# wgurecky/bipymc

Hardware: AMD Instinct MI355X
Metric: chain-updates/sec (higher is better)
Workload: dtype f64

## Files before the change

### bipymc_amd/csrc/kernels.h

```cpp
#pragma once
#ifndef __HIPCC_RTC__
#include <hip/hip_runtime.h>
#include <stdint.h>
#endif

#include "philox.h"

#ifdef BPM_STAMPS
#define BPM_STAMP(i)                                                                          \
    do {                                                                                      \
        __builtin_amdgcn_sched_barrier(0);                                                    \
        unsigned long long _t;                                                                \
        asm volatile("s_memtime %0\n\ts_waitcnt lgkmcnt(0)" : "=s"(_t)::"memory");            \
        __builtin_amdgcn_sched_barrier(0);                                                    \
        bpm_stamp[i] = _t;                                                                    \
    } while (0)
#else
#define BPM_STAMP(i) do { } while (0)
#endif

#if defined(__HIP_DEVICE_COMPILE__) && !defined(__gfx942__) && !defined(__gfx950__)
#error "kernels.h: the ticket hand-overs rely on gfx942 / gfx950 memory behaviour (vmcnt counts stores; agent-scope atomics bypass the L2s): use __ATOMIC_RELEASE / __ATOMIC_ACQUIRE tickets on other targets"
#endif

// ... 459 lines not shown
        }
    }
}

template <int LPC, int DPL>
__device__ __forceinline__ void store_row_sys(double* row, int q, uint32_t ld, const double* v) {
#pragma unroll
    for (int u = 0; u < DPL / 2; ++u) {
        const uint32_t pi = (uint32_t)(q + u * LPC);
        if (2 * pi < ld) {
            __hip_atomic_store(row + 2 * pi, v[2 * u], __ATOMIC_RELAXED, __HIP_MEMORY_SCOPE_SYSTEM);
            __hip_atomic_store(row + 2 * pi + 1, v[2 * u + 1], __ATOMIC_RELAXED, __HIP_MEMORY_SCOPE_SYSTEM);
        }
    }
}

template <int LPC, int DPL>
__device__ __forceinline__ void store_row_stream(double* row, int q, uint32_t ld, const double* v) {
#pragma unroll
    for (int u = 0; u < DPL / 2; ++u) {
        const uint32_t pi = (uint32_t)(q + u * LPC);
        if (2 * pi < ld) {
            bpm_d2v t = {v[2 * u], v[2 * u + 1]};
            __builtin_nontemporal_store(t, reinterpret_cast<bpm_d2v*>(row) + pi);
        }
    }
}

__device__ __forceinline__ void box_muller_pair_f32(uint32_t w1, uint32_t w2, double& n0, double& n1) {
    const float u1 = ((float)w1 + 1.0f) * 2.3283064365386963e-10f;
    const float u2 = (float)w2 * 2.3283064365386963e-10f;
    const float r = __builtin_amdgcn_sqrtf(-2.0f * 0.6931471805599453f * __builtin_amdgcn_logf(u1));
    n0 = (double)(r * __builtin_amdgcn_cosf(u2));
    n1 = (double)(r * __builtin_amdgcn_sinf(u2));
}

template <int K>
__device__ __forceinline__ uint32_t quad_bcast(uint32_t v) {
    return (uint32_t)__builtin_amdgcn_update_dpp(0, (int)v, K * 0x55, 0xF, 0xF, false);
}

template <int LPC, int NPART_CT>
struct Partners {
    uint32_t r[NPART_CT > 0 ? NPART_CT : 1];
    const uint32_t* lds;
    __device__ __forceinline__ uint32_t get(int i) const { return NPART_CT > 0 ? r[i] : lds[i]; }
};

__device__ __forceinline__ uint32_t partner_pos(const PhaseArgs& a, uint32_t c, uint32_t idx, uint32_t n_pair_idx) {
    if (idx < n_pair_idx) {
        const uint32_t p = idx >> 1;
        const u32x4 wb = chain_block(a.seed, c, a.t, SLOT_PAIR0 + (p >> 1));
        uint32_t ia, ib;
        distinct_pair((p & 1) ? wb.z : wb.x, (p & 1) ? wb.w : wb.y, a.M, ia, ib);
        uint32_t pos = (idx & 1) ? ib : ia;
        if (a.mode == 2) pos += (pos >= c) ? 1u : 0u;
        return pos;
    }
    const u32x4 ws = chain_block(a.seed, c, a.t, SLOT_SNK);
    uint32_t iz, i1, i2;
    distinct_three(ws.x, ws.y, ws.z, a.M, iz, i1, i2);
    const uint32_t s = idx - n_pair_idx;
    return s == 0 ? iz : (s == 1 ? i1 : i2);
}

__device__ __forceinline__ uint32_t pos_to_chain(const PhaseArgs& a, uint32_t pos) {
#if defined(BPM_TEST_HOOKS) && defined(BPM_FAKE_NO_PARTNER_HOP)
    return pos;
#else
    return a.perm_tab ? a.perm_tab[pos] : perm_fwd(pos, a.pk);
#endif
}
__device__ __forceinline__ uint32_t own_pos_to_chain(const PhaseArgs& a, uint32_t pos) {
#if defined(BPM_TEST_HOOKS) && defined(BPM_FAKE_NO_OWN_HOP)
    return pos;
#else
    return a.perm_tab ? a.perm_tab[pos] : perm_fwd(pos, a.pk);
#endif
}
__device__ __forceinline__ uint32_t chain_to_pos(const PhaseArgs& a, uint32_t c) {
    return a.inv_tab ? a.inv_tab[c] : perm_inv(c, a.pk);
}

struct NoEarly { template <class W> __device__ __forceinline__ void operator()(W&) const {} };
struct PcrGiven { bool on = false; double p[MAX_CR]; };
template <int ALGO, int LPC, int DPL, int NP, int LOAD_LL = 1 , class EARLY = NoEarly>
__device__ __forceinline__ void make_proposal(const PhaseArgs& a, uint32_t c, bool active, int q, int cw,
                                              uint32_t* s_part, Work<DPL>& wk, const uint32_t* rec = nullptr,
                                              unsigned long long* bpm_stamp = nullptr, EARLY early = EARLY(), const PcrGiven pcr_ovr = PcrGiven()) {
    constexpr bool DREAM = ALGO == ALGO_DREAM;
    constexpr bool FAST = (NP > 0) && (LPC == 1);
    constexpr bool SNK_DIRECT = (LPC == 1);
    const uint32_t dim = a.L.dim, ld = a.L.ld;
    const uint32_t P = NP > 0 ? (uint32_t)NP : a.P;
    load_row<LPC, DPL>(row_ptr(a.L, c), q, ld, wk.x);
    wk.ll_cur = 0.0;
    wk.acc_prev = 0u;
    if (!a.replay) {
#if defined(BPM_TEST_HOOKS) && defined(BPM_FAKE_NO_LL)
        if (LPC < WAVE) wk.ll_cur = wk.x[0] * 1e-300; else
#endif
        if (LOAD_LL == 1 || (LOAD_LL == 2 && !a.lean)) wk.ll_cur = a.ll[c - a.lo];
        if (LPC == WAVE) wk.acc_prev = a.acc_count[c - a.lo];
    }
    if (DREAM && a.adapt_on) {
        load_row<LPC, DPL>(a.w_mean + (uint32_t)((c - a.lo) * 2u * ld), q, ld, wk.w_mean);
        load_row<LPC, DPL>(a.w_m2 + (uint32_t)((c - a.lo) * 2u * ld), q, ld, wk.w_m2);
    }
    double pcr[MAX_CR];
    if (DREAM) {
#pragma unroll
        for (int m = 0; m < MAX_CR; ++m) pcr[m] = pcr_ovr.on ? pcr_ovr.p[m] : a.cr_state[m];
    }
    double gtab[DPL];
    if (DREAM && LPC == WAVE) {
#pragma unroll
        for (int u = 0; u < DPL; ++u) {
            const uint32_t gi = (uint32_t)(q + u * WAVE);
            const double gl = a.gamma_tab[gi <= dim ? gi : dim];
            gtab[u] = gi <= dim ? gl : 0.0;
        }
    }
    double gt_lane = 0.0;
    if (DREAM && LPC * DPL < WAVE) {
        const uint32_t wl = (uint32_t)threadIdx.x & (uint32_t)(WAVE - 1);
        gt_lane = a.gamma_tab[wl <= dim ? wl : dim];
    }
    const bool snk_possible = !DREAM && a.p_snooker > 0.0 && a.M >= 3;
    const uint32_t npart = 2 * P + (snk_possible ? 3u : 0u);
    constexpr bool RL = (LPC == WAVE) && (NP > 0) && !FAST;
    const uint32_t npairs = (dim + 1u) >> 1;
    const bool merged = RL && DPL == 2 && (npairs + 2u * (uint32_t)NP + 1u <= (uint32_t)WAVE);
    u32x4 wpair[DPL / 2];
    u32x4 h0;
    constexpr bool QUAD = DREAM && LPC == 4 && DPL == 2 && NP == 3;
    constexpr bool REGS = FAST || RL || QUAD;
    Partners<LPC, REGS ? 2 * NP : 0> part;
    part.lds = s_part + cw * MAX_PARTNERS;
    const bool planned = (LPC == WAVE) && rec != nullptr;
    const bool dims_late = planned && RL && DPL == 2;
    if (planned) {
        h0.x = rec[1]; h0.y = rec[2]; h0.z = rec[3]; h0.w = rec[4];
        if (FAST || RL) {
#pragma unroll
            for (int i = 0; i < 2 * NP; ++i) part.r[i] = rec[5 + i];
        }
        if (!dims_late) {
#pragma unroll
            for (int u = 0; u < DPL / 2; ++u) wpair[u] = chain_block(a.seed, c, a.t, SLOT_DIM0 + (uint32_t)(q + u * LPC));
        }
    } else if (merged) {
        const uint32_t uq = (uint32_t)q, hdr_lane = npairs + 2u * (uint32_t)NP;
        const uint32_t pidx = uq - npairs;
        const uint32_t slot = uq < npairs ? SLOT_DIM0 + uq : (uq < hdr_lane ? SLOT_PAIR0 + (pidx >> 2) : SLOT_HDR0);
        const u32x4 wb = chain_block(a.seed, c, a.t, slot);
        wpair[0] = wb;
        h0.x = (uint32_t)__builtin_amdgcn_readlane((int)wb.x, hdr_lane);
        h0.y = (uint32_t)__builtin_amdgcn_readlane((int)wb.y, hdr_lane);
        h0.z = (uint32_t)__builtin_amdgcn_readlane((int)wb.z, hdr_lane);
        h0.w = (uint32_t)__builtin_amdgcn_readlane((int)wb.w, hdr_lane);
        BPM_STAMP(2);
        uint32_t mine = 0;
        if (uq >= npairs && uq < hdr_lane) {
            const uint32_t p = pidx >> 1;
            uint32_t ia, ib;
            distinct_pair((p & 1) ? wb.z : wb.x, (p & 1) ? wb.w : wb.y, a.M, ia, ib);
            uint32_t pos = (pidx & 1) ? ib : ia;
            if (a.mode == 2) pos += (pos >= c) ? 1u : 0u;
            mine = pos_to_chain(a, a.pool_off + pos);
        }
#pragma unroll
        for (int i = 0; i < 2 * NP; ++i) part.r[i] = (uint32_t)__builtin_amdgcn_readlane((int)mine, npairs + i);
    } else if (QUAD) {
        wpair[0] = chain_block(a.seed, c, a.t, SLOT_DIM0 + (uint32_t)q);
        const u32x4 wb = chain_block(a.seed, c, a.t, q == 1 ? SLOT_PAIR0 : (q == 2 ? SLOT_PAIR0 + 1u : SLOT_HDR0));
        h0.x = quad_bcast<0>(wb.x); h0.y = quad_bcast<0>(wb.y); h0.z = quad_bcast<0>(wb.z); h0.w = quad_bcast<0>(wb.w);
        uint32_t i0 = 0, i1 = 0, i2 = 0, i3 = 0;
        if (q == 1 || q == 2) {
            uint32_t ia, ib;
            distinct_pair(wb.x, wb.y, a.M, ia, ib);
            i0 = pos_to_chain(a, a.pool_off + ia); i1 = pos_to_chain(a, a.pool_off + ib);
            if (q == 1) {
                distinct_pair(wb.z, wb.w, a.M, ia, ib);
                i2 = pos_to_chain(a, a.pool_off + ia); i3 = pos_to_chain(a, a.pool_off + ib);
            }
        }
        part.r[0] = quad_bcast<1>(i0); part.r[1] = quad_bcast<1>(i1); part.r[2] = quad_bcast<1>(i2); part.r[3] = quad_bcast<1>(i3);
        part.r[4] = quad_bcast<2>(i0); part.r[5] = quad_bcast<2>(i1);
    } else {
        h0 = chain_block(a.seed, c, a.t, SLOT_HDR0);
#pragma unroll
        for (int u = 0; u < DPL / 2; ++u) wpair[u] = chain_block(a.seed, c, a.t, SLOT_DIM0 + (uint32_t)(q + u * LPC));
        if (FAST) {
#pragma unroll
            for (int i = 0; i < 2 * NP; ++i) part.r[i] = pos_to_chain(a, a.pool_off + partner_pos(a, c, (uint32_t)i, 2u * NP));
        }
        if (RL) {
            uint32_t mine = 0;
            if (q < 2 * NP) mine = pos_to_chain(a, a.pool_off + partner_pos(a, c, (uint32_t)q, 2u * NP));
#pragma unroll
            for (int i = 0; i < 2 * NP; ++i) part.r[i] = (uint32_t)__builtin_amdgcn_readlane((int)mine, i);
        }
    }
    BPM_STAMP(3);
    wk.u_acc = u01_53(h0.z, h0.w);
    const double u_sel = (double)(h0.x >> 16) * 1.52587890625e-05;
    const double u_gam = (double)(h0.x & 0xFFFFu) * 1.52587890625e-05;
    uint32_t snk_id[3] = {0u, 0u, 0u};
    if (SNK_DIRECT && snk_possible && planned) {
        snk_id[0] = rec[5 + 2 * P]; snk_id[1] = rec[6 + 2 * P]; snk_id[2] = rec[7 + 2 * P];
    } else if (SNK_DIRECT && snk_possible && (u_sel < a.p_snooker || trace_i32_of(a) != nullptr)) {
        const u32x4 ws = chain_block(a.seed, c, a.t, SLOT_SNK);
        uint32_t iz, i1, i2;
        distinct_three(ws.x, ws.y, ws.z, a.M, iz, i1, i2);
        snk_id[0] = pos_to_chain(a, a.pool_off + iz);
        snk_id[1] = pos_to_chain(a, a.pool_off + i1);
        snk_id[2] = pos_to_chain(a, a.pool_off + i2);
    }
    if (!REGS || (snk_possible && !SNK_DIRECT)) {
#pragma unroll 1
        for (uint32_t idx = (uint32_t)q; idx < npart; idx += LPC)
            s_part[cw * MAX_PARTNERS + idx] = planned ? rec[5 + idx] : pos_to_chain(a, a.pool_off + partner_pos(a, c, idx, 2 * P));
        __builtin_amdgcn_fence(__ATOMIC_RELEASE, "wavefront");
        __builtin_amdgcn_wave_barrier();
        __builtin_amdgcn_fence(__ATOMIC_ACQUIRE, "wavefront");
    }

    constexpr int NPX = NP > 0 ? NP : 1;
    double ra[NPX][DPL], rb[NPX][DPL];
    if (DREAM && NP > 0) {
#pragma unroll
        for (int p = 0; p < NP; ++p) {
            if (LPC == WAVE) {
                load_row_all<LPC, DPL>(row_ptr(a.L, part.get(2 * p)), q, ld, ra[p]);
                load_row_all<LPC, DPL>(row_ptr(a.L, part.get(2 * p + 1)), q, ld, rb[p]);
            } else {
                load_row<LPC, DPL>(row_ptr(a.L, part.get(2 * p)), q, ld, ra[p]);
                load_row<LPC, DPL>(row_ptr(a.L, part.get(2 * p + 1)), q, ld, rb[p]);
            }
        }
    }
    BPM_STAMP(7);
    if (dims_late) wpair[0] = chain_block(a.seed, c, a.t, SLOT_DIM0 + (uint32_t)q);
    if (DREAM) early(wk);

    double eps_n[DPL], eps_u[DPL];
    uint32_t maskbits = 0;
    wk.cr_idx = -1; wk.d_prime = (int)dim; wk.jump = 0; wk.snk = 0; wk.delta = 0.0; wk.log_corr = 0.0;
    uint32_t thr = 65536u;
    if (DREAM) {
        const double uc = u_sel;
        double cum = 0.0;
        int idx = (int)a.n_cr - 1;
        bool found = false;
#pragma unroll
        for (int m = 0; m < MAX_CR; ++m) {
            if (m < (int)a.n_cr) {
                cum += pcr[m];
                if (!found && uc < cum) { idx = m; thr = a.thr[m]; found = true; }
            }
        }
        if (!found) {
#pragma unroll
            for (int m = 0; m < MAX_CR; ++m) if (m == (int)a.n_cr - 1) thr = a.thr[m];
        }
        wk.cr_idx = idx;
    }
    int cnt = 0;
#pragma unroll
    for (int u = 0; u < DPL / 2; ++u) {
        const uint32_t pi = (uint32_t)(q + u * LPC);
        const uint32_t j0 = 2u * pi;
        eps_n[2 * u] = 0.0; eps_n[2 * u + 1] = 0.0; eps_u[2 * u] = 0.0; eps_u[2 * u + 1] = 0.0;
        if (j0 < dim) {
            const u32x4 wj = wpair[u];
            const bool two = j0 + 1 < dim;
            if (a.epsilon > 0.0) {
                double n0, n1;
                box_muller_pair_f32(wj.z, wj.w, n0, n1);
                eps_n[2 * u] = a.epsilon * n0;
                if (two) eps_n[2 * u + 1] = a.epsilon * n1;
            }
            if (DREAM) {
                if (a.u_epsilon > 0.0) {
                    eps_u[2 * u] = -a.u_epsilon + (2.0 * a.u_epsilon) * (((double)(wj.y >> 16) + 0.5) * 1.52587890625e-05);
                    if (two) eps_u[2 * u + 1] = -a.u_epsilon + (2.0 * a.u_epsilon) * (((double)(wj.y & 0xFFFFu) + 0.5) * 1.52587890625e-05);
                }
                if ((wj.x >> 16) <= thr) { maskbits |= 1u << (2 * u); ++cnt; }
                if (two && (wj.x & 0xFFFFu) <= thr) { maskbits |= 1u << (2 * u + 1); ++cnt; }
            }
        }
    }
    if (DREAM) {
        if (LPC == WAVE) {
            cnt = 0;
#pragma unroll
            for (int sb = 0; sb < DPL; ++sb) cnt += (int)__popcll(__ballot((maskbits >> sb) & 1u));
        } else {
            cnt = gsum_i<LPC>(cnt);
        }
        if (cnt == 0) {
            const uint32_t f = mulhi32(h0.y, dim);
#pragma unroll
            for (int s = 0; s < DPL; ++s) {
                const uint32_t j = 2u * (uint32_t)(q + (s >> 1) * LPC) + (s & 1);
                if (j == f) maskbits |= 1u << s;
            }
            cnt = 1;
        }
        wk.d_prime = cnt;
    }
    wk.maskbits = maskbits;

    if (DREAM) {
        double gamma;
        if (LPC == WAVE && (uint32_t)cnt < (uint32_t)(WAVE * DPL)) {
            double gsel = gtab[0];
#pragma unroll
            for (int u = 1; u < DPL; ++u) gsel = ((cnt >> 6) == u) ? gtab[u] : gsel;
            gamma = readlane_f64(gsel, cnt & 63);
        } else if (LPC * DPL < WAVE) {
            gamma = __shfl(gt_lane, cnt);
        } else {
            gamma = a.gamma_tab[cnt];
        }
        if (a.k % 5 == 0 && !(u_gam < 0.2)) { gamma = 1.0; wk.jump = 1; }
        wk.gamma = gamma;
        if (LPC == WAVE) {
            int u_hi = __builtin_amdgcn_readfirstlane(__double2hiint(wk.u_acc)), u_lo = __builtin_amdgcn_readfirstlane(__double2loint(wk.u_acc));
            asm volatile("" : "+s"(u_hi), "+s"(u_lo));
            wk.u_acc = __hiloint2double(u_hi, u_lo);
            asm volatile("" ::"s"(a.wt), "s"(a.hist_by_pos), "s"(a.upd_off), "s"(a.hist_row), "s"(a.llhist_row), "s"(a.ll), "s"(a.acc_count));
        }
        double sum[DPL];
        if (NP > 0) {
#pragma unroll
            for (int s = 0; s < DPL; ++s) {
                sum[s] = ra[0][s] - rb[0][s];
#pragma unroll
                for (int p = 1; p < NP; ++p) sum[s] = sum[s] + (ra[p][s] - rb[p][s]);
            }
        } else {
#pragma unroll
            for (int s = 0; s < DPL; ++s) sum[s] = 0.0;
#pragma unroll 1
            for (uint32_t p = 0; p < P; ++p) {
                double ra[DPL], rb[DPL];
                load_row<LPC, DPL>(row_ptr(a.L, part.lds[2 * p]), q, ld, ra);
                load_row<LPC, DPL>(row_ptr(a.L, part.lds[2 * p + 1]), q, ld, rb);
#pragma unroll
                for (int s = 0; s < DPL; ++s) sum[s] = (p == 0) ? (ra[s] - rb[s]) : (sum[s] + (ra[s] - rb[s]));
            }
        }
#pragma unroll
        for (int s = 0; s < DPL; ++s) {
            const double jump = (1.0 + eps_u[s]) * gamma * sum[s] + eps_n[s];
            wk.p[s] = ((maskbits >> s) & 1u) ? (jump + wk.x[s]) : wk.x[s];
        }
        BPM_STAMP(4);
        if (a.adapt_on && a.cr_gate) {
            const double* m2 = wk.w_m2;
            double dl = 0.0;
#pragma unroll
            for (int s = 0; s < DPL; ++s) {
                const uint32_t j = 2u * (uint32_t)(q + (s >> 1) * LPC) + (s & 1);
                if (j < dim) {
                    const double df = wk.x[s] - wk.p[s];
                    dl += m2[s] > 0.0 ? (df * df * (double)a.hist_len) / m2[s] : (df * df) / 1e-24;
                }
            }
            wk.delta = gsum<LPC>(dl);
        }
    } else {
        double gamma = a.gamma_demc;
        if (a.mode != 2 && a.k % 10 == 0 && !(u_gam < 0.1)) { gamma = 1.0; wk.jump = 1; }
        wk.gamma = gamma;
        double ra[DPL], rb[DPL];
        const bool ids_in_regs = REGS && (!snk_possible || SNK_DIRECT);
        const uint32_t ca = ids_in_regs ? part.get(0) : part.lds[0];
        const uint32_t cb = ids_in_regs ? part.get(1) : part.lds[1];
        const bool do_snk = snk_possible && u_sel < a.p_snooker;
        if (LPC == 1) asm volatile("" ::"v"(ca), "v"(cb), "v"(snk_id[0]), "v"(snk_id[1]), "v"(snk_id[2]));
        load_row<LPC, DPL>(row_ptr(a.L, ca), q, ld, ra);
        load_row<LPC, DPL>(row_ptr(a.L, cb), q, ld, rb);
        double rz[DPL], r1[DPL], r2[DPL];
#pragma unroll
        for (int s = 0; s < DPL; ++s) { rz[s] = 0.0; r1[s] = 0.0; r2[s] = 0.0; }
        if (do_snk) {
            load_row<LPC, DPL>(row_ptr(a.L, SNK_DIRECT ? snk_id[0] : part.lds[2]), q, ld, rz);
            load_row<LPC, DPL>(row_ptr(a.L, SNK_DIRECT ? snk_id[1] : part.lds[3]), q, ld, r1);
            load_row<LPC, DPL>(row_ptr(a.L, SNK_DIRECT ? snk_id[2] : part.lds[4]), q, ld, r2);
        }
        early(wk);
#pragma unroll
        for (int s = 0; s < DPL; ++s) {
            double pv = gamma * (ra[s] - rb[s]);
            pv = pv + wk.x[s];
            pv = pv + eps_n[s];
            wk.p[s] = pv;
        }
        if (do_snk) {
            double n2 = 0.0, dot = 0.0;
#pragma unroll
            for (int s = 0; s < DPL; ++s) {
                const double df = wk.x[s] - rz[s];
                n2 += df * df;
                dot += (r1[s] - r2[s]) * df;
            }
            n2 = gsum<LPC>(n2);
            dot = gsum<LPC>(dot);
            if (n2 > 0.0) {
                const double gs = (1.2 + u01_32(h0.y)) * (dot / n2);
                double n2p = 0.0;
#pragma unroll
                for (int s = 0; s < DPL; ++s) {
                    const uint32_t j = 2u * (uint32_t)(q + (s >> 1) * LPC) + (s & 1);
                    const double df = wk.x[s] - rz[s];
                    double pv = wk.x[s] + gs * df;
                    pv = pv + eps_n[s];
                    if (j >= dim) pv = wk.x[s];
                    wk.p[s] = pv;
                    const double dn = pv - rz[s];
                    n2p += dn * dn;
                }
                n2p = gsum<LPC>(n2p);
                wk.log_corr = 0.5 * (double)(dim - 1) * (log(n2p) - log(n2));
                wk.snk = 1;
            }
        }
    }
    if (trace_i32_of(a) && active) {
        if (q == 0) {
            int32_t* tr = trace_i32_of(a) + (uint64_t)(c - a.lo) * TRACE_I32;
            tr[0] = wk.cr_idx; tr[1] = wk.d_prime; tr[2] = wk.jump; tr[4] = wk.snk;
            if (REGS) {
#pragma unroll
                for (int i = 0; i < 2 * NP; ++i) tr[5 + i] = (int32_t)part.get(i);
            }
            const bool regs = REGS && (!snk_possible || SNK_DIRECT);
#pragma unroll 1
            for (uint32_t i = regs ? 2u * P : 0u; i < MAX_PARTNERS; ++i) {
                int32_t v = -1;
                const uint32_t ks = i - 2u * P;
                if (i < npart) v = regs ? (int32_t)(ks == 1u ? snk_id[1] : (ks == 2u ? snk_id[2] : snk_id[0])) : (int32_t)part.lds[i];
                tr[5 + i] = v;
            }
        }
        if (trace_mask_of(a)) {
#pragma unroll
            for (int s = 0; s < DPL; ++s) {
                const uint32_t j = 2u * (uint32_t)(q + (s >> 1) * LPC) + (s & 1);
                if (j < dim) trace_mask_of(a)[(uint64_t)(c - a.lo) * dim + j] = (uint8_t)((maskbits >> s) & 1u);
            }
        }
    }
}

template <int ALGO, int LPC, int DPL, int LEAN = 0 , bool CRP_W = false>
__device__ __forceinline__ void finish_update(const PhaseArgs& a, uint32_t c, bool active, int q,
                                              const Work<DPL>& wk, double ll_prop) {
    const uint32_t ld = a.L.ld;
    const uint32_t li = c - a.lo;
    const double ll_cur = wk.ll_cur;
    double alpha = exp((ll_prop + wk.log_corr) - ll_cur);
    const bool is_nan = alpha != alpha;
    alpha = fmin(1.0, alpha);
    alpha = fmax(0.0, alpha);
// ... 91 lines not shown
                store_row_stream<LPC, DPL>(a.w_mean + (uint32_t)(li * 2u * ld), q, ld, mean);
                store_row_stream<LPC, DPL>(a.w_m2 + (uint32_t)(li * 2u * ld), q, ld, m2);
            }
        }
        if (q == 0 && a.adapt_on && !(CRP_W && a.cr_part1 != nullptr)) {
            const bool gated = a.adapt_on && a.cr_gate;
            if (a.wt) {
                __hip_atomic_store(delta_ptr(a.L, c), gated ? wk.delta : 0.0, __ATOMIC_RELAXED, __HIP_MEMORY_SCOPE_AGENT);
                __hip_atomic_store(cridx_ptr(a.L, c), gated ? (double)wk.cr_idx : -1.0, __ATOMIC_RELAXED, __HIP_MEMORY_SCOPE_AGENT);
            } else {
                *delta_ptr(a.L, c) = gated ? wk.delta : 0.0;
                *cridx_ptr(a.L, c) = gated ? (double)wk.cr_idx : -1.0;
            }
        }
    }
    if (trace_i32_of(a) && q == 0) {
        trace_i32_of(a)[(uint64_t)li * TRACE_I32 + 3] = accepted ? 1 : 0;
        double* tf = trace_f64_of(a) + (uint64_t)li * TRACE_F64;
        tf[0] = alpha; tf[1] = ll_prop; tf[2] = wk.delta; tf[3] = wk.gamma;
    }
    if (a.n_peers) asm volatile("s_waitcnt vmcnt(0)" ::: "memory");
}

template <int LPC>
__device__ __forceinline__ void pin_args(const PhaseArgs& a) {
    if (LPC != WAVE) {
        asm volatile("" ::"s"(a.L.G), "s"(a.L.ld), "s"(a.L.dim), "s"(a.ll), "s"(a.hist_row), "s"(a.llhist_row), "s"(a.tparams),
                     "s"(a.cr_state), "s"(a.acc_count), "s"(a.perm_tab), "s"(a.inv_tab), "s"(a.gamma_tab), "s"(a.plan), "s"(a.pack),
                     "s"(a.thr[0]), "s"(a.thr[1]), "s"(a.thr[2]), "s"(a.seed), "s"(a.t), "s"(a.k), "s"(a.N),
                     "s"(a.lo), "s"(a.upd_off), "s"(a.n_upd), "s"(a.pool_off), "s"(a.M), "s"(a.mode), "s"(a.n_items), "s"(a.n_cr));
        asm volatile("" ::"s"(a.adapt_on), "s"(a.cr_gate), "s"(a.hist_len), "s"(a.epsilon), "s"(a.u_epsilon), "s"(a.L.n_local),
                     "s"(a.L.world), "s"(a.L.magic), "s"(a.counters), "s"(a.pack_cap), "s"(a.pack_nsub), "s"(a.pack_stride));
    }
}

__device__ __forceinline__ bool resolve_chain(const PhaseArgs& a, uint32_t w, uint32_t& c) {
    bool active = w < a.n_items;
    if (a.mode == 0) {
        c = own_pos_to_chain(a, a.upd_off + (active ? w : 0u));
    } else if (a.mode == 2) {
        c = a.lo + (active ? w : 0u);
    } else {
        c = a.lo + (active ? w : 0u);
        const uint32_t pos = chain_to_pos(a, c);
        active = active && (pos - a.upd_off) < a.n_upd;
    }
    return active;
}

#ifdef BPM_STAMPS
__host__ inline bool stamps_allow_hot(const PhaseArgs&) { return true; }
#else
__host__ inline bool stamps_allow_hot(const PhaseArgs& a) { return a.stamps == nullptr; }
#endif
enum Flavour {
    FLAVOUR_GENERAL = 0,
    FLAVOUR_STEADY_PLAN = 1,
    FLAVOUR_STEADY = 2,
    FLAVOUR_ADAPT_PLAN = 3,
    FLAVOUR_ADAPT = 4,
    FLAVOUR_SHARD_PLAN = 5,
    N_FLAVOURS = 7
};
__host__ inline Flavour choose_flavour(const PhaseArgs& a, bool dream, bool can_plan) {
    const bool plan = can_plan && a.rec_tab != nullptr;
    if (!(a.mode == 0 && (a.rec_tab != nullptr) == plan && trace_i32_of(a) == nullptr && a.pack == nullptr && a.x_next == nullptr && a.epsilon > 0.0 &&
          a.perm_tab != nullptr && a.inv_tab != nullptr && a.replay == 0 && (!dream || (a.u_epsilon > 0.0 && a.n_cr == 3))))
        return FLAVOUR_GENERAL;
    const bool single = a.n_peers == 0 && a.L.world == 1 && a.lo == 0 && stamps_allow_hot(a) && a.accbits == nullptr;
    if (single && a.adapt_on == 0) return plan ? FLAVOUR_STEADY_PLAN : FLAVOUR_STEADY;
    if (plan && a.adapt_on == 0 && a.L.world > 1 && a.stamps == nullptr && (a.accbits != nullptr || a.n_peers > 0)) return FLAVOUR_SHARD_PLAN;
    if (single && a.adapt_on != 0 && dream) return plan ? FLAVOUR_ADAPT_PLAN : FLAVOUR_ADAPT;
    return FLAVOUR_GENERAL;
}
constexpr bool flavour_is_steady(int f) { return f == FLAVOUR_STEADY_PLAN || f == FLAVOUR_STEADY; }
template <int ALGO, int TARGET, int LPC, int DPL, int NP, int HOT = 0>
__global__ __launch_bounds__(block_for_hot(LPC, HOT, DPL)) void phase_fused_kernel(
#ifdef BPM_PRELOAD
    const uint32_t* pl_plan, uint32_t pl_upd_off, uint32_t pl_n_items, uint32_t pl_mode,
#endif
    const PhaseArgs a_in) {
    constexpr bool COPY = (HOT != 0);
    constexpr bool SHARD = (HOT == 5 || HOT == 6), ADAPT = (HOT == 3 || HOT == 4), NOPLAN = (HOT == 2 || HOT == 4 || HOT == 6);
    PhaseArgs a_hot;
    if (COPY) {
        a_hot = a_in;
        a_hot.mode = 0u; trace_set(a_hot, nullptr, nullptr, nullptr); a_hot.pack = nullptr;
        a_hot.replay = 0u; a_hot.x_next = nullptr; a_hot.adapt_on = ADAPT ? 1u : 0u;
#ifndef BPM_STAMPS
        a_hot.stamps = nullptr;
#else
        if (SHARD) a_hot.stamps = nullptr;
#endif
        if (!ADAPT) a_hot.cr_fold_part = nullptr;
        if (!SHARD) { a_hot.accbits = nullptr; a_hot.lo = 0; a_hot.L.world = 1; a_hot.acc_by_item = 0u; a_hot.n_peers = 0u; a_hot.peer_tab = nullptr; }
        if (ALGO == ALGO_DREAM) a_hot.n_cr = 3;
        if (NOPLAN) { a_hot.plan = nullptr; a_hot.rec_tab = nullptr; }
    }
    const PhaseArgs& a = COPY ? a_hot : a_in;
    if (HOT) {
        __builtin_assume(a_in.mode == 0u); __builtin_assume(a_in.pack == nullptr);
#ifdef BPM_TEST_HOOKS
        __builtin_assume(a_in.trace_i32 == nullptr);
#endif
        __builtin_assume(a_in.x_next == nullptr); __builtin_assume(a_in.adapt_on == (ADAPT ? 1u : 0u));
#ifndef BPM_STAMPS
        __builtin_assume(a_in.stamps == nullptr);
#endif
        if (!SHARD) { __builtin_assume(a_in.lo == 0); __builtin_assume(a_in.L.world == 1); }
        __builtin_assume(a_in.epsilon > 0.0);
        __builtin_assume(a_in.perm_tab != nullptr); __builtin_assume(a_in.inv_tab != nullptr);
        if (ALGO == ALGO_DREAM) { __builtin_assume(a_in.u_epsilon > 0.0); __builtin_assume(a_in.n_cr == 3); }
    }
#ifdef BPM_PRELOAD
    if (HOT) { __builtin_assume(pl_mode == 0u); __builtin_assume((pl_plan != nullptr) == !NOPLAN); }
#else
    const uint32_t* pl_plan = a.rec_tab;
    const uint32_t pl_upd_off = a.rec_off, pl_n_items = a.n_items, pl_mode = a.mode;
#endif
    constexpr int BLK = block_for_hot(LPC, HOT, DPL);
    constexpr bool CRP = ALGO == ALGO_DREAM && hot_is_adapt(HOT) && crp_shape(LPC, DPL);
    __shared__ uint32_t s_part[(BLK / LPC) * MAX_PARTNERS];
    const int lane = threadIdx.x;
    const int cw = lane / LPC, q = lane % LPC;
    const uint32_t w = blockIdx.x * (BLK / LPC) + cw;
#ifdef BPM_STAMPS
    unsigned long long bpm_stamp[8] = {0, 0, 0, 0, 0, 0, 0, 0};
    unsigned long long bpm_rt0;
    asm volatile("s_memrealtime %0\n\ts_waitcnt lgkmcnt(0)" : "=s"(bpm_rt0)::"memory");
    BPM_STAMP(0);
#endif
    pin_args<LPC>(a);
    uint32_t c;
    bool active;
    const uint32_t* rec = nullptr;
    bool run = true;
    double cr_d = 0.0;
    int cr_i = -1;
    if (LPC == WAVE && pl_plan && !(CRP && w >= pl_n_items)) {
        active = w < pl_n_items;
        if (!active) return;
        uint32_t pos;
        if (pl_mode == 0) {
            pos = pl_upd_off + w;
        } else {
            pos = a.inv_tab[a.lo + w];
            if ((pos - pl_upd_off) >= a.n_upd) return;
        }
        pos = __builtin_amdgcn_readfirstlane(pos);
        rec = pl_plan + (uint32_t)(pos * PLAN_WORDS);
        c = rec[0];
    } else {
        active = resolve_chain(a, w, c);
    }
    if (LPC == WAVE && !active) {
        if (CRP) run = false; else return;
    }
    PcrGiven pcr_fold;
    if constexpr (CRP) {
        pcr_fold.on = a.cr_fold_part != nullptr;
        if (pcr_fold.on) {
            __shared__ double s_tot[2 * MAX_CR];
            constexpr uint32_t NWV = (uint32_t)(BLK / WAVE);
            const uint32_t n_cr = a.n_cr, wv = (uint32_t)lane / (uint32_t)WAVE;
            for (uint32_t k = wv; k < 2u * n_cr; k += NWV) {
                const uint32_t arr = k < n_cr ? k : (uint32_t)MAX_CR + (k - n_cr);
                const double tsum = cr_array_sum<CR_FINAL_MAX / WAVE>(a.cr_fold_part + (uint64_t)arr * a.cr_fold_nb, a.cr_fold_nb);
                if ((lane & (WAVE - 1)) == 0) s_tot[arr] = tsum;
            }
            __syncthreads();
            CrTotals T;
#pragma unroll
            for (int m = 0; m < MAX_CR; ++m) { T.p[m] = a.cr_fold_tot[m]; T.d[m] = a.cr_fold_tot[MAX_CR + m]; T.n[m] = a.cr_fold_tot[2 * MAX_CR + m]; }
            bool any = false;
#pragma unroll
            for (int m = 0; m < MAX_CR; ++m) {
                if (m < (int)n_cr) {
                    const double td = s_tot[m], tn = s_tot[MAX_CR + m];
                    if (tn > 0.0) { any = true; T.n[m] += tn; T.d[m] += td; }
                }
            }
            cr_finalize(any, n_cr, T);
            if (blockIdx.x == 0 && lane == 0) cr_write_totals(T, n_cr, a.cr_fold_out);
#pragma unroll
            for (int m = 0; m < MAX_CR; ++m)
                pcr_fold.p[m] = __hiloint2double(__builtin_amdgcn_readfirstlane(__double2hiint(T.p[m])), __builtin_amdgcn_readfirstlane(__double2loint(T.p[m])));
        }
    }
  if (run) {
    if (LPC == WAVE) c = __builtin_amdgcn_readfirstlane(c);
    const typename Target<TARGET, LPC, DPL>::Consts tc = Target<TARGET, LPC, DPL>::load(q, a.L.dim, a.tparams);
    Work<DPL> wk;
    wk.item = w;
    wk.pos_own = a.upd_off + (active ? w : 0u);
    if (LPC == WAVE) wk.pos_own = (uint32_t)__builtin_amdgcn_readfirstlane((int)wk.pos_own);
    constexpr bool LEAN = lean_scalars<TARGET, LPC>();
    const uint32_t dim_early = a.L.dim;
    constexpr bool LEAN_CT = LEAN && lean_always<TARGET>();
#ifdef BPM_STAMPS
    bpm_stamp[1] = 0; BPM_STAMP(1);
    unsigned long long* const stamp_arg = bpm_stamp;
#else
    unsigned long long* const stamp_arg = nullptr;
#endif
    if constexpr (LEAN) {
        const bool lean_early = LEAN_CT || a.lean != 0u;
        auto early = [tc, q, dim_early, lean_early](Work<DPL>& k) { if (lean_early) k.ll_cur = Target<TARGET, LPC, DPL>::eval(k.x, q, dim_early, tc); };
        make_proposal<ALGO, LPC, DPL, NP, (LEAN_CT ? 0 : 2)>(a, c, active, q, cw, s_part, wk, rec, stamp_arg, early, pcr_fold);
    } else if constexpr (CRP) {
        make_proposal<ALGO, LPC, DPL, NP>(a, c, active, q, cw, s_part, wk, rec, stamp_arg, NoEarly(), pcr_fold);
    } else {
        make_proposal<ALGO, LPC, DPL, NP>(a, c, active, q, cw, s_part, wk, rec, stamp_arg);
    }
    const double ll_prop = Target<TARGET, LPC, DPL>::eval(wk.p, q, a.L.dim, tc);
    BPM_STAMP(5);
    finish_update<ALGO, LPC, DPL, (LEAN_CT ? 2 : (LEAN ? 1 : 0)), CRP>(a, c, active, q, wk, ll_prop);
    if (CRP && active && a.adapt_on && a.cr_gate) { cr_d = wk.delta; cr_i = wk.cr_idx; }
    BPM_STAMP(6);
#ifdef BPM_STAMPS
    if (bpm_stamp[2] == 0) { bpm_stamp[2] = bpm_rt0; bpm_stamp[1] = bpm_stamp[7]; }
    {
        unsigned long long rt;
        asm volatile("s_memrealtime %0\n\ts_waitcnt lgkmcnt(0)" : "=s"(rt)::"memory");
        bpm_stamp[7] = (rt & 0x0FFFFFFFFFFFFFFFull) | ((unsigned long long)(__builtin_amdgcn_s_getreg((31 << 11) | 20) & 0xF) << 60);
    }
    if (a.stamps && lane == 0) for (int i = 0; i < 8; ++i) a.stamps[(uint64_t)w * 8 + i] = bpm_stamp[i];
#endif
  }
    if (CRP && a.cr_part1) {
        constexpr int G1 = cr_g1(LPC);
        if (LPC == WAVE) {
            __shared__ double s_crd[G1];
            __shared__ int s_cri[G1];
            if (q == 0) { s_crd[cw] = cr_d; s_cri[cw] = cr_i; }
            __syncthreads();
            if (cw == 0 && q < (int)a.n_cr) {
                double sd = 0.0, sn = 0.0;
#pragma unroll
                for (int k = 0; k < G1; ++k) cr_chunk_add(sd, sn, q, s_cri[k], s_crd[k]);
                const uint32_t ch = a.cr_chunk0 + blockIdx.x;
                __hip_atomic_store(&a.cr_part1[(uint64_t)q * a.cr_n1 + ch], sd, __ATOMIC_RELAXED, __HIP_MEMORY_SCOPE_AGENT);
                __hip_atomic_store(&a.cr_part1[(uint64_t)(MAX_CR + q) * a.cr_n1 + ch], sn, __ATOMIC_RELAXED, __HIP_MEMORY_SCOPE_AGENT);
            }
        } else {
            const int wl = lane & (WAVE - 1);
            double sd = 0.0, sn = 0.0;
#pragma unroll
            for (int k = 0; k < G1; ++k) {
                const double dk = readlane_f64(cr_d, k * LPC);
                const int ik = __builtin_amdgcn_readlane(cr_i, k * LPC);
                cr_chunk_add(sd, sn, wl, ik, dk);
            }
            const uint32_t ch = a.cr_chunk0 + (blockIdx.x * (BLK / WAVE) + (uint32_t)(lane / WAVE));
            if (wl < (int)a.n_cr && (ch - a.cr_chunk0) * (uint32_t)G1 < a.n_items) {
                __hip_atomic_store(&a.cr_part1[(uint64_t)wl * a.cr_n1 + ch], sd, __ATOMIC_RELAXED, __HIP_MEMORY_SCOPE_AGENT);
                __hip_atomic_store(&a.cr_part1[(uint64_t)(MAX_CR + wl) * a.cr_n1 + ch], sn, __ATOMIC_RELAXED, __HIP_MEMORY_SCOPE_AGENT);
            }
        }
    }
}

template <int ALGO, int LPC, int DPL, int NP>
__global__ __launch_bounds__(block_for(LPC)) void phase_replay_kernel(const PhaseArgs a_in) {
    PhaseArgs a_rep;
    if (LPC == WAVE) {
        a_rep = a_in;
        a_rep.replay = 1u; a_rep.adapt_on = 0u; trace_set(a_rep, nullptr, nullptr, nullptr);
        a_rep.pack = nullptr; a_rep.x_next = nullptr; a_rep.stamps = nullptr; a_rep.mode = 1u; a_rep.n_peers = 0u;
    }
    const PhaseArgs& a = (LPC == WAVE) ? a_rep : a_in;
    __shared__ uint32_t s_part[(block_for(LPC) / LPC) * MAX_PARTNERS];
    const int lane = threadIdx.x;
    const int cw = lane / LPC, q = lane % LPC;
    const uint32_t w = blockIdx.x * (block_for(LPC) / LPC) + cw;
    bool active = w < a.n_upd;
    uint32_t pos = a.upd_off + (active ? w : 0u);
    const uint32_t* rec = nullptr;
    uint32_t c;
    if (LPC == WAVE && a.plan) {
        if (!active) return;
        pos = __builtin_amdgcn_readfirstlane(pos);
        rec = a.plan + (uint32_t)(pos * PLAN_WORDS);
        c = rec[0];
    } else {
        c = pos_to_chain(a, pos);
    }
    active = active && (c - a.lo) >= a.L.n_local && a.accbits_all[c] != 0;
    if (LPC == WAVE && !active) return;
    if (LPC == WAVE) c = __builtin_amdgcn_readfirstlane(c);
    Work<DPL> wk;
    make_proposal<ALGO, LPC, DPL, NP>(a, c, active, q, cw, s_part, wk, rec);
    if (active) store_row<LPC, DPL>(row_ptr(a.L, c), q, a.L.ld, wk.p);
}

#ifndef BPM_REPLAY_WG
// ... 862 lines not shown
```

Before: 780.9 million.

## Issue planned-record and row loads at kernel entry before argument copy

For hot wavefront-per-chain kernels with a plan, the kernel now reads the 64-byte plan record as one vector load at entry, then immediately issues loads for the own row, partner rows, log-likelihood, acceptance count, CR probabilities, gamma table and target constants. These are held in a PlanFront struct, and make_proposal consumes them instead of reloading. The aim is to start dependent global loads earlier and overlap their latency with argument-block setup. Empty asm constraints pin scalars and sched barriers fix the ordering, which adds register pressure and code complexity.

Measured after the change: 790.5 million (median of 6 runs). 1.01x the previous value.

```diff
diff --git a/bipymc_amd/csrc/kernels.h b/bipymc_amd/csrc/kernels.h
--- a/bipymc_amd/csrc/kernels.h
+++ b/bipymc_amd/csrc/kernels.h
@@ -565,17 +565,49 @@
     return a.inv_tab ? a.inv_tab[c] : perm_inv(c, a.pk);
 }
 
+template <int DPL, int NPX>
+struct PlanFront {
+    uint32_t rec[PLAN_WORDS];
+    double x[DPL], ra[NPX][DPL], rb[NPX][DPL];
+    double ll_cur, pcr[3], gl[DPL];
+    uint32_t acc_prev;
+};
+typedef uint32_t bpm_u32x16 __attribute__((ext_vector_type(16)));
+__device__ __forceinline__ bpm_u32x16 plan_record(const uint32_t* recp) {
+    return *reinterpret_cast<const bpm_u32x16*>(__builtin_assume_aligned(recp, 4 * PLAN_WORDS));
+}
+template <int DPL, int NP>
+__device__ __forceinline__ void plan_front(const Layout& L, const bpm_u32x16 rv, int q, PlanFront<DPL, (NP > 0 ? NP : 1)>& fr) {
+    static_assert(PLAN_WORDS == 16 && DPL == 2, "one 64-byte record, one 16-byte load per lane and row");
+#pragma unroll
+    for (int i = 0; i < PLAN_WORDS; ++i) fr.rec[i] = rv[i];
+    load_row_all<WAVE, DPL>(row_ptr(L, fr.rec[0]), q, L.ld, fr.x);
+#pragma unroll
+    for (int p = 0; p < NP; ++p) {
+        load_row_all<WAVE, DPL>(row_ptr(L, fr.rec[5 + 2 * p]), q, L.ld, fr.ra[p]);
+        load_row_all<WAVE, DPL>(row_ptr(L, fr.rec[5 + 2 * p + 1]), q, L.ld, fr.rb[p]);
+    }
+    __builtin_amdgcn_sched_barrier(0);
+}
+
 struct NoEarly { template <class W> __device__ __forceinline__ void operator()(W&) const {} };
 struct PcrGiven { bool on = false; double p[MAX_CR]; };
-template <int ALGO, int LPC, int DPL, int NP, int LOAD_LL = 1 , class EARLY = NoEarly>
+template <int ALGO, int LPC, int DPL, int NP, int LOAD_LL = 1 , class EARLY = NoEarly, bool FRONT = false>
 __device__ __forceinline__ void make_proposal(const PhaseArgs& a, uint32_t c, bool active, int q, int cw,
                                               uint32_t* s_part, Work<DPL>& wk, const uint32_t* rec = nullptr,
-                                              unsigned long long* bpm_stamp = nullptr, EARLY early = EARLY(), const PcrGiven pcr_ovr = PcrGiven()) {
+                                              unsigned long long* bpm_stamp = nullptr, EARLY early = EARLY(), const PcrGiven pcr_ovr = PcrGiven(),
+                                              const PlanFront<DPL, (NP > 0 ? NP : 1)>* fr = nullptr) {
+    static_assert(!FRONT || (LPC == WAVE && DPL == 2), "the planned front serves one wavefront per chain with one coordinate pair per lane");
     constexpr bool DREAM = ALGO == ALGO_DREAM;
     constexpr bool FAST = (NP > 0) && (LPC == 1);
     constexpr bool SNK_DIRECT = (LPC == 1);
     const uint32_t dim = a.L.dim, ld = a.L.ld;
     const uint32_t P = NP > 0 ? (uint32_t)NP : a.P;
+    if constexpr (FRONT) {
+        const bool in_row = 2u * (uint32_t)q < ld;
+#pragma unroll
+        for (int s = 0; s < DPL; ++s) wk.x[s] = in_row ? fr->x[s] : 0.0;
+    } else
     load_row<LPC, DPL>(row_ptr(a.L, c), q, ld, wk.x);
     wk.ll_cur = 0.0;
     wk.acc_prev = 0u;
@@ -583,7 +615,9 @@
 #if defined(BPM_TEST_HOOKS) && defined(BPM_FAKE_NO_LL)
         if (LPC < WAVE) wk.ll_cur = wk.x[0] * 1e-300; else
 #endif
+        if constexpr (FRONT) wk.ll_cur = fr->ll_cur; else
         if (LOAD_LL == 1 || (LOAD_LL == 2 && !a.lean)) wk.ll_cur = a.ll[c - a.lo];
+        if constexpr (FRONT) wk.acc_prev = fr->acc_prev; else
         if (LPC == WAVE) wk.acc_prev = a.acc_count[c - a.lo];
     }
     if (DREAM && a.adapt_on) {
@@ -593,14 +627,15 @@
     double pcr[MAX_CR];
     if (DREAM) {
 #pragma unroll
-        for (int m = 0; m < MAX_CR; ++m) pcr[m] = pcr_ovr.on ? pcr_ovr.p[m] : a.cr_state[m];
+        for (int m = 0; m < MAX_CR; ++m)
+            pcr[m] = pcr_ovr.on ? pcr_ovr.p[m] : (FRONT ? (m < 3 ? fr->pcr[m < 3 ? m : 0] : 0.0) : a.cr_state[m]);
     }
     double gtab[DPL];
     if (DREAM && LPC == WAVE) {
 #pragma unroll
         for (int u = 0; u < DPL; ++u) {
             const uint32_t gi = (uint32_t)(q + u * WAVE);
-            const double gl = a.gamma_tab[gi <= dim ? gi : dim];
+            const double gl = FRONT ? fr->gl[u] : a.gamma_tab[gi <= dim ? gi : dim];
             gtab[u] = gi <= dim ? gl : 0.0;
         }
     }
@@ -613,16 +648,24 @@
     const uint32_t npart = 2 * P + (snk_possible ? 3u : 0u);
     constexpr bool RL = (LPC == WAVE) && (NP > 0) && !FAST;
     const uint32_t npairs = (dim + 1u) >> 1;
-    const bool merged = RL && DPL == 2 && (npairs + 2u * (uint32_t)NP + 1u <= (uint32_t)WAVE);
+    const bool merged = !FRONT && RL && DPL == 2 && (npairs + 2u * (uint32_t)NP + 1u <= (uint32_t)WAVE);
     u32x4 wpair[DPL / 2];
     u32x4 h0;
     constexpr bool QUAD = DREAM && LPC == 4 && DPL == 2 && NP == 3;
     constexpr bool REGS = FAST || RL || QUAD;
     Partners<LPC, REGS ? 2 * NP : 0> part;
     part.lds = s_part + cw * MAX_PARTNERS;
-    const bool planned = (LPC == WAVE) && rec != nullptr;
+    const bool planned = FRONT || ((LPC == WAVE) && rec != nullptr);
     const bool dims_late = planned && RL && DPL == 2;
-    if (planned) {
+    if (FRONT) {
+        h0.x = fr->rec[1]; h0.y = fr->rec[2]; h0.z = fr->rec[3]; h0.w = fr->rec[4];
+#pragma unroll
+        for (int i = 0; i < 2 * NP; ++i) part.r[i] = fr->rec[5 + i];
+        if (!dims_late) {
+#pragma unroll
+            for (int u = 0; u < DPL / 2; ++u) wpair[u] = chain_block(a.seed, c, a.t, SLOT_DIM0 + (uint32_t)(q + u * LPC));
+        }
+    } else if (planned) {
         h0.x = rec[1]; h0.y = rec[2]; h0.z = rec[3]; h0.w = rec[4];
         if (FAST || RL) {
 #pragma unroll
@@ -711,7 +754,13 @@
 
     constexpr int NPX = NP > 0 ? NP : 1;
     double ra[NPX][DPL], rb[NPX][DPL];
-    if (DREAM && NP > 0) {
+    if (FRONT && DREAM && NP > 0) {
+#pragma unroll
+        for (int p = 0; p < NP; ++p) {
+#pragma unroll
+            for (int s = 0; s < DPL; ++s) { ra[p][s] = fr->ra[p][s]; rb[p][s] = fr->rb[p][s]; }
+        }
+    } else if (DREAM && NP > 0) {
 #pragma unroll
         for (int p = 0; p < NP; ++p) {
             if (LPC == WAVE) {
@@ -723,7 +772,7 @@
             }
         }
     }
-    BPM_STAMP(7);
+    if (!FRONT) BPM_STAMP(7);
     if (dims_late) wpair[0] = chain_block(a.seed, c, a.t, SLOT_DIM0 + (uint32_t)q);
     if (DREAM) early(wk);
 
@@ -864,8 +913,14 @@
         const uint32_t cb = ids_in_regs ? part.get(1) : part.lds[1];
         const bool do_snk = snk_possible && u_sel < a.p_snooker;
         if (LPC == 1) asm volatile("" ::"v"(ca), "v"(cb), "v"(snk_id[0]), "v"(snk_id[1]), "v"(snk_id[2]));
+        if constexpr (FRONT && NP == 1) {
+            const bool in_row = 2u * (uint32_t)q < ld;
+#pragma unroll
+            for (int s = 0; s < DPL; ++s) { ra[s] = in_row ? fr->ra[0][s] : 0.0; rb[s] = in_row ? fr->rb[0][s] : 0.0; }
+        } else {
         load_row<LPC, DPL>(row_ptr(a.L, ca), q, ld, ra);
         load_row<LPC, DPL>(row_ptr(a.L, cb), q, ld, rb);
+        }
         double rz[DPL], r1[DPL], r2[DPL];
 #pragma unroll
         for (int s = 0; s < DPL; ++s) { rz[s] = 0.0; r1[s] = 0.0; r2[s] = 0.0; }
@@ -1123,41 +1178,12 @@
     const PhaseArgs a_in) {
     constexpr bool COPY = (HOT != 0);
     constexpr bool SHARD = (HOT == 5 || HOT == 6), ADAPT = (HOT == 3 || HOT == 4), NOPLAN = (HOT == 2 || HOT == 4 || HOT == 6);
-    PhaseArgs a_hot;
-    if (COPY) {
-        a_hot = a_in;
-        a_hot.mode = 0u; trace_set(a_hot, nullptr, nullptr, nullptr); a_hot.pack = nullptr;
-        a_hot.replay = 0u; a_hot.x_next = nullptr; a_hot.adapt_on = ADAPT ? 1u : 0u;
-#ifndef BPM_STAMPS
-        a_hot.stamps = nullptr;
-#else
-        if (SHARD) a_hot.stamps = nullptr;
-#endif
-        if (!ADAPT) a_hot.cr_fold_part = nullptr;
-        if (!SHARD) { a_hot.accbits = nullptr; a_hot.lo = 0; a_hot.L.world = 1; a_hot.acc_by_item = 0u; a_hot.n_peers = 0u; a_hot.peer_tab = nullptr; }
-        if (ALGO == ALGO_DREAM) a_hot.n_cr = 3;
-        if (NOPLAN) { a_hot.plan = nullptr; a_hot.rec_tab = nullptr; }
-    }
-    const PhaseArgs& a = COPY ? a_hot : a_in;
-    if (HOT) {
-        __builtin_assume(a_in.mode == 0u); __builtin_assume(a_in.pack == nullptr);
-#ifdef BPM_TEST_HOOKS
-        __builtin_assume(a_in.trace_i32 == nullptr);
-#endif
-        __builtin_assume(a_in.x_next == nullptr); __builtin_assume(a_in.adapt_on == (ADAPT ? 1u : 0u));
-#ifndef BPM_STAMPS
-        __builtin_assume(a_in.stamps == nullptr);
-#endif
-        if (!SHARD) { __builtin_assume(a_in.lo == 0); __builtin_assume(a_in.L.world == 1); }
-        __builtin_assume(a_in.epsilon > 0.0);
-        __builtin_assume(a_in.perm_tab != nullptr); __builtin_assume(a_in.inv_tab != nullptr);
-        if (ALGO == ALGO_DREAM) { __builtin_assume(a_in.u_epsilon > 0.0); __builtin_assume(a_in.n_cr == 3); }
-    }
+    constexpr bool FRONT_CT = LPC == WAVE && DPL == 2 && (HOT == 1 || HOT == 3 || HOT == 5);
 #ifdef BPM_PRELOAD
     if (HOT) { __builtin_assume(pl_mode == 0u); __builtin_assume((pl_plan != nullptr) == !NOPLAN); }
 #else
-    const uint32_t* pl_plan = a.rec_tab;
-    const uint32_t pl_upd_off = a.rec_off, pl_n_items = a.n_items, pl_mode = a.mode;
+    const uint32_t* pl_plan = (HOT && NOPLAN) ? nullptr : a_in.rec_tab;
+    const uint32_t pl_upd_off = a_in.rec_off, pl_n_items = a_in.n_items, pl_mode = HOT ? 0u : a_in.mode;
 #endif
     constexpr int BLK = block_for_hot(LPC, HOT, DPL);
     constexpr bool CRP = ALGO == ALGO_DREAM && hot_is_adapt(HOT) && crp_shape(LPC, DPL);
@@ -1171,6 +1197,114 @@
     asm volatile("s_memrealtime %0\n\ts_waitcnt lgkmcnt(0)" : "=s"(bpm_rt0)::"memory");
     BPM_STAMP(0);
 #endif
+    PlanFront<DPL, (NP > 0 ? NP : 1)> fr;
+    uint32_t f_c = 0u;
+    const uint32_t* f_rec = nullptr;
+    Layout f_L = {};
+    double *f_ll = nullptr, *f_wm = nullptr, *f_w2 = nullptr;
+    const double *f_crs = nullptr, *f_tp = nullptr, *f_gt = nullptr;
+    uint32_t* f_acc = nullptr;
+    unsigned long long* f_cnt = nullptr;
+    uint32_t f_lo = 0u;
+    typename Target<TARGET, LPC, DPL>::Consts tc_front;
+    if constexpr (FRONT_CT) {
+        if (w < pl_n_items) {
+            f_L = a_in.L;
+            if (SHARD) __builtin_assume(f_L.world > 1u); else f_L.world = 1;
+            typedef uint32_t u32x4_a4 __attribute__((ext_vector_type(4), aligned(4)));
+            typedef uint32_t u32x2_a4 __attribute__((ext_vector_type(2), aligned(4)));
+            u32x4_a4 lw4 = {0u, 0u, 0u, 0u};
+            u32x2_a4 lw2 = {0u, 0u};
+            if (SHARD) {
+                lw4 = *reinterpret_cast<const u32x4_a4*>(&a_in.L.n_local);
+                lw2 = *reinterpret_cast<const u32x2_a4*>(&a_in.L.magic);
+                f_L.n_local = lw4.x; f_L.ld = lw4.y; f_L.dim = lw4.z; f_L.world = lw4.w; f_L.magic = lw2.x;
+                __builtin_assume(f_L.world > 1u);
+            }
+            f_ll = a_in.ll; f_acc = a_in.acc_count; f_crs = a_in.cr_state; f_tp = a_in.tparams; f_gt = a_in.gamma_tab; f_cnt = a_in.counters;
+            if (ADAPT) { f_wm = a_in.w_mean; f_w2 = a_in.w_m2; }
+            if (SHARD) f_lo = a_in.lo;
+            const uint32_t pos = (uint32_t)__builtin_amdgcn_readfirstlane((int)(pl_upd_off + w));
+            f_rec = pl_plan + (uint32_t)(pos * PLAN_WORDS);
+            bpm_u32x16 rv = plan_record(f_rec);
+#ifndef BPM_STAMPS
+#define BPM_FRONT_ALL "s"(f_L.G), "s"(f_L.ld), "s"(f_L.dim), "s"(f_ll), "s"(f_acc), "s"(f_tp), "s"(f_cnt), "s"(a_in.seed), "s"(a_in.t), "s"(a_in.k), "s"(a_in.upd_off), \
+                      "s"(a_in.epsilon), "s"(a_in.wt), "s"(a_in.hist_by_pos), "s"(a_in.hist_row), "s"(a_in.llhist_row)
+#define BPM_FRONT_DREAM "s"(f_crs), "s"(f_gt), "s"(a_in.u_epsilon), "s"(a_in.thr[0]), "s"(a_in.thr[1]), "s"(a_in.thr[2]), "s"(a_in.thr[3])
+            if (ALGO == ALGO_DREAM && ADAPT) asm("" : "+s"(rv) : BPM_FRONT_ALL, BPM_FRONT_DREAM, "s"(f_wm), "s"(f_w2), "s"(a_in.cr_gate), "s"(a_in.hist_len));
+            else if (ALGO == ALGO_DREAM && SHARD) asm("" : "+s"(rv) : BPM_FRONT_ALL, BPM_FRONT_DREAM, "s"(f_lo), "s"(lw4), "s"(lw2));
+            else if (ALGO == ALGO_DREAM) asm("" : "+s"(rv) : BPM_FRONT_ALL, BPM_FRONT_DREAM);
+            else if (SHARD) asm("" : "+s"(rv) : BPM_FRONT_ALL, "s"(a_in.gamma_demc), "s"(a_in.p_snooker), "s"(a_in.M), "s"(a_in.pool_off), "s"(f_lo), "s"(lw4), "s"(lw2));
+            else asm("" : "+s"(rv) : BPM_FRONT_ALL, "s"(a_in.gamma_demc), "s"(a_in.p_snooker), "s"(a_in.M), "s"(a_in.pool_off));
+#undef BPM_FRONT_ALL
+#undef BPM_FRONT_DREAM
+#endif
+            __builtin_amdgcn_sched_barrier(0);
+            f_c = rv[0];
+            fr.ll_cur = f_ll[f_c - f_lo];
+            fr.acc_prev = f_acc[f_c - f_lo];
+            if (ALGO == ALGO_DREAM) {
+#pragma unroll
+                for (int m = 0; m < 3; ++m) fr.pcr[m] = f_crs[m];
+#pragma unroll
+                for (int u = 0; u < DPL; ++u) {
+                    const uint32_t gi = (uint32_t)(q + u * WAVE);
+                    fr.gl[u] = f_gt[gi <= f_L.dim ? gi : f_L.dim];
+                }
+            }
+            tc_front = Target<TARGET, LPC, DPL>::load(q, f_L.dim, f_tp);
+            plan_front<DPL, NP>(f_L, rv, q, fr);
+#ifndef BPM_STAMPS
+            if constexpr (ALGO == ALGO_DREAM && TARGET == TARGET_GAUSS)
+                asm("" : "+s"(f_c) : "s"(fr.ll_cur), "s"(fr.acc_prev), "s"(fr.pcr[0]), "s"(fr.pcr[1]), "s"(fr.pcr[2]), "s"(tc_front.c0), "s"(tc_front.a), "s"(tc_front.b));
+            else if (ALGO == ALGO_DREAM) asm("" : "+s"(f_c) : "s"(fr.ll_cur), "s"(fr.acc_prev), "s"(fr.pcr[0]), "s"(fr.pcr[1]), "s"(fr.pcr[2]));
+            else if constexpr (TARGET == TARGET_GAUSS) asm("" : "+s"(f_c) : "s"(fr.ll_cur), "s"(fr.acc_prev), "s"(tc_front.c0), "s"(tc_front.a), "s"(tc_front.b));
+            else asm("" : "+s"(f_c) : "s"(fr.ll_cur), "s"(fr.acc_prev));
+#endif
+#ifdef BPM_STAMPS
+            BPM_STAMP(7);
+#endif
+        } else if (!CRP) {
+            return;
+        }
+    }
+    PhaseArgs a_hot;
+    if (COPY) {
+        if constexpr (FRONT_CT) {
+            a_hot = a_in;
+            a_hot.L = f_L; a_hot.ll = f_ll; a_hot.acc_count = f_acc; a_hot.cr_state = f_crs; a_hot.tparams = f_tp; a_hot.gamma_tab = f_gt; a_hot.counters = f_cnt;
+            if (ADAPT) { a_hot.w_mean = f_wm; a_hot.w_m2 = f_w2; }
+            if (SHARD) a_hot.lo = f_lo;
+        } else
+        a_hot = a_in;
+        a_hot.mode = 0u; trace_set(a_hot, nullptr, nullptr, nullptr); a_hot.pack = nullptr;
+        a_hot.replay = 0u; a_hot.x_next = nullptr; a_hot.adapt_on = ADAPT ? 1u : 0u;
+#ifndef BPM_STAMPS
+        a_hot.stamps = nullptr;
+#else
+        if (SHARD) a_hot.stamps = nullptr;
+#endif
+        if (!ADAPT) a_hot.cr_fold_part = nullptr;
+        if (!SHARD) { a_hot.accbits = nullptr; a_hot.lo = 0; a_hot.L.world = 1; a_hot.acc_by_item = 0u; a_hot.n_peers = 0u; a_hot.peer_tab = nullptr; }
+        if (ALGO == ALGO_DREAM) a_hot.n_cr = 3;
+        if (NOPLAN) { a_hot.plan = nullptr; a_hot.rec_tab = nullptr; }
+    }
+    const PhaseArgs& a = COPY ? a_hot : a_in;
+    static_assert(!FRONT_CT || COPY, "the planned front reads the argument block through the private copy");
+    if (HOT) {
+        __builtin_assume(a_in.mode == 0u); __builtin_assume(a_in.pack == nullptr);
+#ifdef BPM_TEST_HOOKS
+        __builtin_assume(a_in.trace_i32 == nullptr);
+#endif
+        __builtin_assume(a_in.x_next == nullptr); __builtin_assume(a_in.adapt_on == (ADAPT ? 1u : 0u));
+#ifndef BPM_STAMPS
+        __builtin_assume(a_in.stamps == nullptr);
+#endif
+        if (!SHARD) { __builtin_assume(a_in.lo == 0); __builtin_assume(a_in.L.world == 1); }
+        __builtin_assume(a_in.epsilon > 0.0);
+        __builtin_assume(a_in.perm_tab != nullptr); __builtin_assume(a_in.inv_tab != nullptr);
+        if (ALGO == ALGO_DREAM) { __builtin_assume(a_in.u_epsilon > 0.0); __builtin_assume(a_in.n_cr == 3); }
+    }
     pin_args<LPC>(a);
     uint32_t c;
     bool active;
@@ -1178,7 +1312,11 @@
     bool run = true;
     double cr_d = 0.0;
     int cr_i = -1;
-    if (LPC == WAVE && pl_plan && !(CRP && w >= pl_n_items)) {
+    if constexpr (FRONT_CT) {
+        active = w < pl_n_items;
+        c = f_c;
+        rec = f_rec;
+    } else if (LPC == WAVE && pl_plan && !(CRP && w >= pl_n_items)) {
         active = w < pl_n_items;
         if (!active) return;
         uint32_t pos;
@@ -1230,7 +1368,7 @@
     }
   if (run) {
     if (LPC == WAVE) c = __builtin_amdgcn_readfirstlane(c);
-    const typename Target<TARGET, LPC, DPL>::Consts tc = Target<TARGET, LPC, DPL>::load(q, a.L.dim, a.tparams);
+    const typename Target<TARGET, LPC, DPL>::Consts tc = FRONT_CT ? tc_front : Target<TARGET, LPC, DPL>::load(q, a.L.dim, a.tparams);
     Work<DPL> wk;
     wk.item = w;
     wk.pos_own = a.upd_off + (active ? w : 0u);
@@ -1249,9 +1387,9 @@
         auto early = [tc, q, dim_early, lean_early](Work<DPL>& k) { if (lean_early) k.ll_cur = Target<TARGET, LPC, DPL>::eval(k.x, q, dim_early, tc); };
         make_proposal<ALGO, LPC, DPL, NP, (LEAN_CT ? 0 : 2)>(a, c, active, q, cw, s_part, wk, rec, stamp_arg, early, pcr_fold);
     } else if constexpr (CRP) {
-        make_proposal<ALGO, LPC, DPL, NP>(a, c, active, q, cw, s_part, wk, rec, stamp_arg, NoEarly(), pcr_fold);
+        make_proposal<ALGO, LPC, DPL, NP, 1, NoEarly, FRONT_CT>(a, c, active, q, cw, s_part, wk, rec, stamp_arg, NoEarly(), pcr_fold, &fr);
     } else {
-        make_proposal<ALGO, LPC, DPL, NP>(a, c, active, q, cw, s_part, wk, rec, stamp_arg);
+        make_proposal<ALGO, LPC, DPL, NP, 1, NoEarly, FRONT_CT>(a, c, active, q, cw, s_part, wk, rec, stamp_arg, NoEarly(), PcrGiven(), &fr);
     }
     const double ll_prop = Target<TARGET, LPC, DPL>::eval(wk.p, q, a.L.dim, tc);
     BPM_STAMP(5);
```
